# lingya/titan

Hardware: AMD Instinct MI355X
Metric: BFS GTEPS + PageRank s/iter, RMAT scale-24 (1 GPU) and scale-27 (1/2/4/8 GPU) (higher is better)
Workload: dtype int32 (BFS levels); f64 (PageRank)

## Files before the change

titan_amd/csrc/api_msbfs.cpp:

```cpp
#include <algorithm>
#include <cstdio>
#include <cstring>
#include "ctx.hpp"

using namespace tgo;

namespace tgo {

int ms_alloc(tgo_ctx* ctx) {
    Scratch& s = ctx->sc;
    if (s.ms_vis) return TGO_OK;
    const int64_t n = ctx->g.n;
    HIP_TRY(dev_alloc(ctx, s.ms_vis, n + 1));
    HIP_TRY(dev_alloc(ctx, s.ms_fr, n + 1));
    HIP_TRY(dev_alloc(ctx, s.ms_nx, n + 1));
    HIP_TRY(dev_alloc(ctx, s.ms_lvl, n * kLevelPlanes + 1));
    s.ms_clean = 0;
    if (n > ctx->g.n_active)
        for (int k = 0; k < kLevelPlanes; ++k)
            HIP_TRY(hipMemsetAsync(s.ms_lvl + static_cast<int64_t>(k) * n + ctx->g.n_active, 0,
                                   (n - ctx->g.n_active) * sizeof(uint64_t), ctx->stream));
    HIP_TRY(dev_alloc(ctx, s.ms_fbm, (n + 63) / 64 + 1));
    HIP_TRY(dev_alloc(ctx, s.ms_seeds, TGO_MAX_SOURCES));
    HIP_TRY(dev_alloc(ctx, s.ms_stat, 2 * TGO_MAX_SOURCES));
    HIP_TRY(dev_alloc(ctx, s.ms_srcent, TGO_MAX_SOURCES));
    ctx->st.device_bytes = ctx->dev_bytes;
    return TGO_OK;
}

double ms_split_of(const tgo_ctx* ctx) {
    static const double env = env_double("TGO_MS_SPLIT", 0.005);
    return tuned(ctx->tune.f64(TGO_TUNE_MS_SPLIT), env);
}
double ms_stay_of(const tgo_ctx* ctx) {
    static const double env = env_clamped("TGO_MS_STAY", kMsStayDefault, 0.0, HUGE_VAL);
    return tuned(ctx->tune.f64(TGO_TUNE_MS_STAY), env);
}
double ms_sparse_of(const tgo_ctx* ctx) {
    static const double env = env_clamped("TGO_MS_SPARSE", kMsSparseDefault, 0.0, HUGE_VAL);
    return tuned(ctx->tune.f64(TGO_TUNE_MS_SPARSE), env);
}
int64_t ms_head_of(const tgo_ctx* ctx) {
    static const int64_t env = static_cast<int64_t>(
        env_clamped("TGO_MS_HEAD", static_cast<double>(kMsHeadDefault), 0.0, static_cast<double>(kMsHeadMax)));
    return tuned(ctx->tune.i64(TGO_TUNE_MS_HEAD), env);
}

}

static int ms_cold_layout(tgo_ctx* ctx, int32_t scope, const View& pull, int64_t hot_req) {
    DevGraph& g = ctx->g;
    Scratch& s = ctx->sc;
    static const int64_t hot_env = static_cast<int64_t>(env_double("TGO_MS_COLD_HOT", 393216.0));
    static const int64_t seg_env = static_cast<int64_t>(env_double("TGO_MS_COLD_SEG", 393216.0));
    const int64_t hot = hot_req > 1 ? hot_req : hot_env, seg = hot_req > 1 ? hot_req : seg_env;
    if (g.msc_scope == scope && g.msc_req == hot) return TGO_OK;
// ... 10 lines not shown
    if (C == 0) return TGO_OK;
    adopt(ctx, g.msc_adj, cadj);
    adopt(ctx, g.msc_row, crow);
    if (!s.ms_cacc) {
        HIP_TRY(dev_alloc(ctx, s.ms_cacc, g.n + 1));
        HIP_TRY(dev_alloc(ctx, s.ms_need, g.n + 1));
        HIP_TRY(hipMemsetAsync(s.ms_need, 0, g.n + 1, ctx->stream));
    }
    g.msc_C = C;
    g.msc_hot = static_cast<int32_t>(hot);
    ctx->st.device_bytes = ctx->dev_bytes;
    return TGO_OK;
}

namespace tgo {

int run_ms_sweep(tgo_ctx* ctx, const int64_t* in, int32_t nseeds, int32_t max_depth, int32_t scope, int32_t flags) {
    int rc = TGO_OK;
    DevGraph& g = ctx->g;
    Scratch& s = ctx->sc;
    hipStream_t st = ctx->stream;
    const int64_t n = g.n;
    const View pull = pull_view(g, scope), push = push_view(g, scope);
    std::vector<int32_t> uniq;
    for (int r = 0; r < nseeds; ++r)
        if (std::find(uniq.begin(), uniq.end(), static_cast<int32_t>(in[r])) == uniq.end())
            uniq.push_back(static_cast<int32_t>(in[r]));
    s.ms_nsrc = nseeds;
    HIP_TRY(hipEventRecord(ctx->ev0, st));
    HIP_TRY(hipMemcpyAsync(s.ms_seeds, in, nseeds * sizeof(int64_t), hipMemcpyHostToDevice, st));
    HIP_TRY(hipMemcpyAsync(s.q[0], uniq.data(), uniq.size() * sizeof(int32_t), hipMemcpyHostToDevice, st));
    HIP_TRY(hipMemsetAsync(s.ms_vis, 0, n * 8, st));
    const bool masks_zero = s.ms_masks_zero;
    s.ms_masks_zero = false;
    if (!masks_zero) HIP_TRY(hipMemsetAsync(s.ms_fr, 0, n * 8, st));
    s.ms_nplanes = 0;
    HIP_TRY(k_ms_seed(s.ms_seeds, nseeds, s.ms_vis, s.ms_fr, INT64_MAX, st));
    HIP_TRY(k_degree_i64(push, s.q[0], static_cast<int64_t>(uniq.size()), s.qdeg, st));
    const uint64_t full = nseeds == 64 ? ~0ULL : ((1ULL << nseeds) - 1ULL);
    const int64_t total = pull.nlists > 1 ? g.out.nnz + g.in.nnz : (scope == TGO_SCOPE_IN_E ? g.out.nnz : g.in.nnz);
    static const double ms_alpha = env_double("TGO_MS_ALPHA", 12.0);
    static const bool trace = trace_on();
    static const int32_t filter_from = env_double("TGO_MS_FILTER", 0.0) != 0.0
        ? 0 : static_cast<int32_t>(env_double("TGO_MS_FILTER_FROM", -1.0));
    const bool filter = filter_from >= 0 && filter_from < n;
    const double split_frac = tgo::ms_split_of(ctx);
    const double stay_gamma = tgo::ms_stay_of(ctx), sparse_frac = tgo::ms_sparse_of(ctx);
    const int64_t head = tgo::ms_head_of(ctx);
    static const bool diag = env_double("TGO_MS_DIAG", 0.0) != 0.0;
    static const bool compact_on = env_i64("TGO_MS_COMPACT", 1) != 0 && !diag;
    static const int32_t compact_chunk = [] {
        const int64_t c = env_i64("TGO_MS_CHUNK", kMsChunkDefault);
        return static_cast<int32_t>(c == 512 || c == 1024 || c == 2048 ? c : kMsChunkDefault);
    }();
    int64_t qlen = static_cast<int64_t>(uniq.size());
    int64_t mf = 0;
    int64_t reached = qlen;
    bool srcent_ready = false;
    static const double push_light = env_double("TGO_MS_PUSH_LIGHT", 1.0 / 16.0);
    static const bool push_probe = env_double("TGO_MS_PUSH_PROBE", 1.0) != 0.0;
    static const int push_range_log2 = static_cast<int>(env_double("TGO_MS_PUSH_RANGE", 0.0));
    static const int64_t push_range_min = static_cast<int64_t>(env_double("TGO_MS_PUSH_RANGE_MIN", 1048576.0));
    const int depth = std::min(max_depth, 65534);
    uint64_t* fr = s.ms_fr;
    uint64_t* nx = s.ms_nx;
    int cur = 0, levels = 0;
    bool queued = true;
    bool pulled = false;
    bool cnt_zero = false;
    bool nx_clean = masks_zero;
    int64_t prev_mf = 0;
    int64_t mu = -1;
    bool level0_sparse = false, last_sparse = false;
    unsigned long long se_pub[TGO_MAX_SOURCES] = {};
    const volatile unsigned long long* hw = host_words(ctx);
    for (int L = 0; L < depth && qlen > 0; ++L) {
        const bool stay = pulled && mu >= 0 && stay_gamma > 0.0 &&
                          static_cast<double>(mu) <= stay_gamma * static_cast<double>(mf);
        const bool use_pull = stay || static_cast<double>(mf) * ms_alpha > static_cast<double>(total);
        DevSpan span(st, "msbfs.level", {"level", L}, {"pull", use_pull ? 1 : 0}, {"compact", 0});
        if ((rc = ms_planes_for(ctx, L + 1, true))) return rc;
        const uint32_t was_clean = s.ms_clean & ms_planes_written(L + 1);
        s.ms_clean &= ~was_clean;
        const bool queued_before = queued;
        if (!use_pull && !queued) {
            if (!cnt_zero) HIP_TRY(hipMemsetAsync(s.cnt, 0, sizeof(Counters), st));
            HIP_TRY(k_ms_queue(push, g.n_active, fr, s.q[cur], s.qdeg, s.cnt, st));
        }
        queued = !use_pull;
        const bool prev_pull = pulled;
        pulled = use_pull;
        bool sums = false;
        if (!use_pull && !queued_before) cnt_zero = false;
        bool sparse_level = false;
        bool count_open = false;
        if (use_pull) {
            if (!cnt_zero) HIP_TRY(hipMemsetAsync(s.cnt, 0, sizeof(Counters), st));
            cnt_zero = true;
            uint64_t sparse = 0;
            if (split_frac > 0.0 && !prev_pull) {
                static const bool srcent_check = env_double("TGO_MS_SRCENT_CHECK", 0.0) != 0.0;
                if (srcent_ready && srcent_check) {
                    HIP_TRY(k_ms_source_entries(push, fr, g.n_active, full, s.ms_stat, st));
                    unsigned long long x[TGO_MAX_SOURCES];
                    HIP_TRY(hipMemcpyAsync(x, s.ms_stat, sizeof(x), hipMemcpyDeviceToHost, st));
                    HIP_TRY(hipStreamSynchronize(st));
// ... 15 lines not shown
                std::sort(order, order + nseeds, [&](int a, int b) { return se[a] < se[b]; });
                const double budget = split_frac * static_cast<double>(total);
                double used = 0.0;
                for (int i = 0; i < nseeds; ++i) {
                    const int r = order[i];
                    if (used + static_cast<double>(se[r]) > budget) break;
                    used += static_cast<double>(se[r]);
                    sparse |= 1ULL << r;
                }
                if (sparse == full) sparse = 0;
                if (sparse) {
                    bool any = false;
                    for (int r = 0; r < nseeds; ++r) any |= ((sparse >> r) & 1ULL) && se[r] > 0;
                    if (!nx_clean) HIP_TRY(hipMemsetAsync(nx, 0, g.n_active * 8, st));
                    if (any) {
                        HIP_TRY(k_ms_queue(push, g.n_active, fr, s.q[cur ^ 1], s.qdeg, s.cnt, st, sparse));
                        if ((rc = turn(ctx))) return rc;
                        const int64_t sq = static_cast<int64_t>(s.hcnt->qlen);
                        if (sq > 0) {
                            if ((rc = scan_frontier(ctx, sq))) return rc;
                            HIP_TRY(k_ms_push(push, s.q[cur ^ 1], s.qpre, sq, fr, s.ms_vis, nx, st, PackTouch{}, sparse));
                        }
                    }
                    if (trace) std::fprintf(stderr, "[tgo] ms level %d split: %d sparse sources, %.0f push entries\n", L,
                                            __builtin_popcountll(sparse), used);
                }
            }
            if (filter) HIP_TRY(k_ms_fbitmap(fr, n, s.ms_fbm, st));
            MsColdSplit cs;
            static const bool cold_env = env_double("TGO_MS_COLD", 0.0) != 0.0;
            const int64_t cold = ctx->tune.i64(TGO_TUNE_MS_COLD);
            const bool cold_on = tuned_on(cold, cold_env);
            if (cold_on && !prev_pull && !filter) {
                if ((rc = ms_cold_layout(ctx, scope, pull, cold))) return rc;
                if (g.msc_C > 0) {
                    cs.hot_lim = g.msc_hot;
                    cs.acc = s.ms_cacc;
                    cs.need = s.ms_need;
                }
            }
            count_open = stay_gamma > 0.0 && !cs.acc && mf < prev_mf;
            const bool compact = compact_on && count_open && !sparse;
            if (compact) span.set_third(1);
            HIP_TRY(k_ms_pull(pull, push, g.n_active, full, fr, filter ? s.ms_fbm : nullptr, s.ms_vis, nx,
                              ms_planes(ctx), s.cnt, L + 1, st, filter ? filter_from : 0, full & ~sparse,
                              sparse ? nx : nullptr, cs, count_open, cs.acc ? 0 : head,
                              compact ? compact_chunk : 0));
            if (cs.acc) {
                HIP_TRY(k_ms_cold(g.msc_adj, g.msc_row, g.msc_C, fr, s.ms_need, s.ms_cacc, st));
                HIP_TRY(k_ms_finish(push, g.n_active, full, s.ms_vis, nx, sparse ? nx : nullptr, ms_planes(ctx), s.cnt,
                                    L + 1, s.ms_need, s.ms_cacc, st));
            }
        } else {
            HIP_TRY(k_level_prep(cnt_zero ? nullptr : s.cnt, nx, nx_clean ? 0 : g.n_active, s.qdeg + qlen, st));
            cnt_zero = true;
            const int64_t rng = static_cast<int64_t>(1) << std::min(40, std::max(0, push_range_log2));
            const int64_t nr = (g.n_active + rng - 1) / rng;
            const bool ranged = push_range_log2 > 0 && mf >= push_range_min && nr > 1 &&
                                (nr + 1) * qlen <= kMsRangePairs && nr * qlen + 1 <= n + 2;
            sparse_level = sparse_frac > 0.0 && !ranged &&
                           (L == 0 || static_cast<double>(mf) <= sparse_frac * static_cast<double>(g.n_active));
            sums = split_frac > 0.0 && (L == 0 || static_cast<double>(mf) * ms_alpha * 64.0 > static_cast<double>(total));
            if (ranged) {
                for (int b = 0; b < 2; ++b)
                    if (!s.ms_rp[b]) HIP_TRY(dev_alloc(ctx, s.ms_rp[b], kMsRangePairs));
                const bool light = static_cast<double>(reached) < push_light * static_cast<double>(n);
                HIP_TRY(k_ms_push_ranged(push, s.q[cur], qlen, g.n_active, rng, s.ms_rp[0], s.ms_rp[1], s.qdeg, s.qpre,
                                         s.cub_tmp, s.cub_bytes, fr, light ? nullptr : s.ms_vis, nx, st));
            } else {
            HIP_TRY(scan_exclusive_i64(s.cub_tmp, s.cub_bytes, s.qdeg, s.qpre, qlen + 1, st));
            if (sparse_level)
                HIP_TRY(k_ms_push_sparse(push, s.q[cur], s.qpre, qlen, fr, s.ms_vis, nx, s.q[cur ^ 1], s.cnt, st));
            else {
            const bool light = static_cast<double>(reached) < push_light * static_cast<double>(n);
            HIP_TRY(k_ms_push(push, s.q[cur], s.qpre, qlen, fr, light ? nullptr : s.ms_vis, nx, st, PackTouch{}, ~0ULL,
                              light ? push_probe : true));
            }
            }
            if (sums && !s.ms_srcent_zero) HIP_TRY(hipMemsetAsync(s.ms_srcent, 0, 64 * sizeof(unsigned long long), st));
            if (sums) s.ms_srcent_zero = false;
            const bool next_pull = static_cast<double>(mf) * ms_alpha * 8.0 > static_cast<double>(total);
            if (sparse_level) {
                HIP_TRY(k_ms_settle_sparse(push, s.q[cur ^ 1], s.qdeg, s.ms_vis, nx, ms_planes(ctx), s.cnt, L + 1, st,
                                           sums ? s.ms_srcent : nullptr, s.q[cur], qlen, fr));
            } else if (next_pull) {
                HIP_TRY(k_ms_settle_count(push, g.n_active, s.ms_vis, nx, ms_planes(ctx), s.cnt, L + 1, st,
                                          sums ? s.ms_srcent : nullptr));
                queued = false;
            } else {
                HIP_TRY(k_ms_settle(push, g.n_active, s.ms_vis, nx, ms_planes(ctx), s.q[cur ^ 1], s.qdeg, s.cnt, L + 1,
                                    st, sums ? s.ms_srcent : nullptr));
            }
        }
        srcent_ready = !use_pull && sums;
        {
            unsigned long long seq = 0;
            if ((rc = turn_begin(ctx, seq, sums ? s.ms_srcent : nullptr))) return rc;
            cnt_zero = true;
            if (sums) s.ms_srcent_zero = true;
            if (L + 1 < depth && (rc = ms_planes_for(ctx, L + 2, true))) return rc;
            if ((rc = wait_publish(ctx, seq))) return rc;
        }
        qlen = static_cast<int64_t>(s.hcnt->qlen);
        if (qlen == 0) s.ms_clean |= was_clean;
        prev_mf = mf;
        mf = static_cast<int64_t>(s.hcnt->mf);
        mu = count_open ? static_cast<int64_t>(s.hcnt->open) : -1;
        if (sums)
            for (int r = 0; r < TGO_MAX_SOURCES; ++r) se_pub[r] = hw[kPublishExtra + r];
        reached += qlen;
        nx_clean = sparse_level;
        last_sparse = sparse_level;
        if (L == 0) level0_sparse = sparse_level;
        if (trace) std::fprintf(stderr, "[tgo] ms level %d %s -> %lld vertices, %lld entries, %llu source-bits%s\n", L,
                                use_pull ? "pull" : "push", (long long)qlen, (long long)mf, s.hcnt->red[0],
                                use_pull ? (stay ? " (stayed in pull)" : "") : (sparse_level ? " (sparse)" : ""));
        if (trace && count_open) std::fprintf(stderr, "[tgo]   %lld list entries of still-open vertices\n", (long long)mu);
        if (trace && diag && use_pull) {
            unsigned long long d[kMsDiagWords] = {};
            HIP_TRY(k_ms_diag_take(d, st));
            std::fprintf(stderr, "[tgo]   pull: %llu entries examined, %llu hot / %llu cold mask gathers, %llu open vertices, "
                         "%llu stopped early; long lists: %llu, %llu entries examined (%llu hot / %llu cold gathers), "
                         "%llu stopped early\n", d[0], d[1], d[2], d[3], d[4], d[6], d[5], d[8], d[9], d[7]);
            std::fprintf(stderr, "[tgo]   long lists covered within 4 / 8 / 16 / 32 / 64 entries: %llu / %llu / %llu / %llu / %llu, "
                         "later %llu, never %llu (head %lld)\n", d[10], d[11], d[12], d[13], d[14], d[15], d[16],
                         static_cast<long long>(head));
        }
        std::swap(fr, nx);
        cur ^= 1;
        ++levels;
    }
    if (qlen > 0 && max_depth > depth)
        return fail(ctx, TGO_E_UNSUPPORTED, "multi-source BFS stores levels as uint16: depth > 65534");
    if (int rc = program_end(ctx, max_depth)) return rc;
    ctx->st.levels = levels;
    s.ms_masks_zero = level0_sparse && last_sparse && qlen == 0;
    if (flags & TGO_FLAG_STATS) {
        HIP_TRY(hipMemsetAsync(s.ms_stat, 0, 2 * TGO_MAX_SOURCES * sizeof(unsigned long long), st));
        HIP_TRY(k_ms_reach(pull, s.ms_vis, n, nseeds, s.ms_stat, s.ms_stat + TGO_MAX_SOURCES, st));
        HIP_TRY(hipStreamSynchronize(st));
    }
    return TGO_OK;
}

// ... 61 lines not shown
```

titan_amd/csrc/engine.hpp:

```cpp
#pragma once
#include <algorithm>
#include <cstdint>
#include <string>
#include <vector>
#include <hip/hip_runtime_api.h>
#include "../../include/titan_gpu_olap.h"
#include "env.hpp"

namespace tgo {

template <class T>
struct DevArray {
    T* p = nullptr;
    int64_t n = -1;
    DevArray() = default;
    DevArray(const DevArray&) = delete;
    DevArray& operator=(const DevArray&) = delete;
    DevArray(DevArray&& o) noexcept : p(o.p), n(o.n) { o.p = nullptr; o.n = -1; }
    DevArray& operator=(DevArray&& o) noexcept {
        if (this != &o) { reset(); p = o.p; n = o.n; o.p = nullptr; o.n = -1; }
        return *this;
    }
    ~DevArray() { reset(); }
    void reset() { if (p) (void)hipFree(p); p = nullptr; n = -1; }
// ... 621 lines not shown
                          const unsigned long long* offs, unsigned long long* cursor, int64_t* send, hipStream_t s);
hipError_t k_ds_mark_sizes(unsigned long long* counts, int nranks, int64_t qlen, unsigned long long* offs,
                           unsigned long long* cursor, const long long* track, int64_t* sizes, hipStream_t s);
hipError_t k_ds_apply(const View& push, const int64_t* recv, int64_t npairs, int64_t* dist, uint64_t* pend, int32_t* qn,
                      int64_t* qdeg_n, Counters* cnt, int64_t thr, const int64_t* ws_off, const int64_t* light,
                      long long* track, hipStream_t s);
hipError_t k_unpermute_i64(const int64_t* in, const int32_t* perm, int64_t* out, int64_t n, hipStream_t s);
hipError_t k_ms_seed(const int64_t* seeds, int nseeds, uint64_t* vis, uint64_t* fr, int64_t fr_rows, hipStream_t s);
constexpr int kMsDiagWords = 17;
hipError_t k_ms_diag_take(unsigned long long* out, hipStream_t s);
hipError_t k_ms_pull(const View& pull, const View& push, int64_t n_active, uint64_t full, const uint64_t* fr,
                     const uint64_t* fbm, uint64_t* vis, uint64_t* nx, LevelPlanes lvl, Counters* cnt,
                     int32_t next_level, hipStream_t s, int32_t filter_from, uint64_t dense = ~0ULL,
                     const uint64_t* cand = nullptr, MsColdSplit cs = MsColdSplit(), bool count_open = false,
                     int64_t head = 0, int32_t compact_chunk = 0);
hipError_t k_ms_cold(const int32_t* cadj, const int32_t* crow, int64_t C, const uint64_t* fr, const uint8_t* need,
                     uint64_t* acc, hipStream_t s);
hipError_t k_ms_finish(const View& push, int64_t n_active, uint64_t full, uint64_t* vis, uint64_t* nx,
                       const uint64_t* cand, LevelPlanes lvl, Counters* cnt, int32_t next_level, uint8_t* need,
                       const uint64_t* acc, hipStream_t s);
hipError_t k_cold_flags(const int32_t* adj, int64_t m, int32_t hot, uint32_t* flag, hipStream_t s);
hipError_t k_cold_emit(const int64_t* off, int64_t n, const int32_t* adj, int64_t m, const uint32_t* flag,
                       const uint64_t* pos, int64_t base, int32_t hot, int64_t seg, uint64_t* key, int32_t* val,
                       hipStream_t s);
hipError_t k_low_rows(const uint64_t* key, int64_t m, int32_t* row, hipStream_t s);
int build_ms_cold(const View& v, int64_t n, int32_t hot, int64_t seg, DevArray<int32_t>& cadj, DevArray<int32_t>& crow,
                  int64_t& C, hipStream_t s, std::string& err);
hipError_t k_ms_source_counts(const uint64_t* fr, int64_t n_active, unsigned long long* out64, hipStream_t s);
hipError_t k_ms_source_entries(const View& push, const uint64_t* fr, int64_t n_active, uint64_t cand,
                               unsigned long long* out64, hipStream_t s);
hipError_t k_ms_fbitmap(const uint64_t* fr, int64_t n, uint64_t* fbm, hipStream_t s);
hipError_t k_ms_queue(const View& push, int64_t n_active, const uint64_t* fr, int32_t* qn, int64_t* qdeg, Counters* cnt,
                      hipStream_t s, uint64_t mask = ~0ULL);
struct PackTouch { uint8_t* flag = nullptr; int64_t n_local = 1; int64_t cps = 1; };
hipError_t k_ms_push(const View& push, const int32_t* q, const int64_t* qpre, int64_t qlen, const uint64_t* fr,
                     const uint64_t* vis, uint64_t* nx, hipStream_t s, PackTouch touch = {}, uint64_t mask = ~0ULL,
                     bool probe = true, uint64_t* own_nx = nullptr, int64_t own_lo = 0);
constexpr double kMsStayDefault = 4.0;
constexpr double kMsSparseDefault = 1.0 / 16.0;
constexpr int64_t kMsHeadDefault = 4;
constexpr int64_t kMsHeadMax = 1 << 20;
constexpr int64_t kMsChunkDefault = 1024;
hipError_t k_ms_push_sparse(const View& push, const int32_t* q, const int64_t* qpre, int64_t qlen, const uint64_t* fr,
                            const uint64_t* vis, uint64_t* nx, int32_t* qn, Counters* cnt, hipStream_t s);
hipError_t k_ms_settle_sparse(const View& push, const int32_t* qn, int64_t* qdeg, uint64_t* vis, const uint64_t* nx,
                              LevelPlanes lvl, Counters* cnt, int32_t next_level, hipStream_t s,
                              unsigned long long* srcent, const int32_t* qp, int64_t qplen, uint64_t* fr);
constexpr int64_t kMsRangePairs = int64_t(1) << 22;
hipError_t k_ms_push_ranged(const View& push, const int32_t* q, int64_t qlen, int64_t n_active, int64_t S,
                            int64_t* P0, int64_t* P1, int64_t* cnt, int64_t* pre, void*& tmp, size_t& tmp_bytes,
                            const uint64_t* fr, const uint64_t* vis, uint64_t* nx, hipStream_t s, uint64_t mask = ~0ULL);
hipError_t k_ms_settle_count(const View& push, int64_t n_active, uint64_t* vis, uint64_t* nx, LevelPlanes lvl,
                            Counters* cnt, int32_t next_level, hipStream_t s, unsigned long long* srcent = nullptr);
hipError_t k_ms_settle(const View& push, int64_t n_active, uint64_t* vis, uint64_t* nx, LevelPlanes lvl, int32_t* qn,
                       int64_t* qdeg, Counters* cnt, int32_t next_level, hipStream_t s,
                       unsigned long long* srcent = nullptr);
hipError_t k_ms_reach(const View& v, const uint64_t* vis, int64_t n_active, int nsrc, unsigned long long* reached,
                      unsigned long long* entries, hipStream_t s);
hipError_t k_ms_extract(LevelPlanes lvl, int nplanes, const uint64_t* vis, const int32_t* perm, int r, int64_t* dist,
                        int64_t n, hipStream_t s);
hipError_t k_or_slices(const uint64_t* recv, int nslices, int64_t n_local, uint64_t* out, hipStream_t s);
constexpr int64_t kPackChunk = 2048;
hipError_t k_ms_pack(bool write, uint64_t* cand, int64_t n_local, int64_t cps, int64_t nchunks, int64_t* cnt,
                     const int64_t* offs, int64_t* send, hipStream_t s, uint8_t* touched = nullptr, int self = -1);
hipError_t k_ms_or_local(uint64_t* cand_own, int64_t n_local, int64_t cps, uint8_t* touched_own, uint64_t* nx,
                         hipStream_t s);
hipError_t k_slice_elems(const int64_t* off, int64_t cps, int nranks, int64_t* out, hipStream_t s);
hipError_t k_ms_or_pairs(const int64_t* pairs, int64_t npairs, uint64_t* nx, hipStream_t s);
hipError_t k_ms_pack_fixed(uint64_t* cand, int64_t n_local, int64_t cps, int64_t nchunks, const int64_t* offs,
                           int nranks, int64_t cap, int64_t* send, int* ovf, uint8_t* touched, hipStream_t s,
                           int self = -1);
hipError_t k_ms_or_fixed(const int64_t* recv, int nslices, int64_t cap, uint64_t* nx, hipStream_t s);
hipError_t k_part_td_mark(const View& push, const int32_t* q, const int64_t* qpre, int64_t qlen,
                          uint64_t* disc, const uint64_t* vb_local, int64_t lo, int64_t n_local, hipStream_t s);
hipError_t k_part_claim(const View& push, const uint64_t* recv, int nslices, int64_t words, int64_t n_local,
                        uint64_t* vb, uint64_t* nb, int32_t* level, int32_t* qn, int64_t* qdeg_n,
                        Counters* cnt, int32_t next_level, hipStream_t s, bool or_into_nb = false);
hipError_t k_part_td_claim(const View& push, const int32_t* q, const int64_t* qpre, int64_t qlen, uint64_t* disc,
                           uint64_t* vb, uint64_t* nb, int32_t* level, int32_t* qn, int64_t* qdeg_n, Counters* cnt,
                           int32_t next_level, int64_t lo, int64_t n_local, hipStream_t s);
int part_bfs_td_fused(tgo_ctx* ctx, int32_t level, uint64_t* disc, uint64_t* nb_local);
int part_bfs_claim_remote(tgo_ctx* ctx, int32_t level, const uint64_t* recv, int32_t nslices, uint64_t* nb_local);
int part_bfs_level_done(tgo_ctx* ctx);
hipError_t k_unpermute_i32(const int32_t* in, const int32_t* perm, int32_t* out, int64_t n, hipStream_t s);

hipError_t k_cc_init(int32_t* parent, int64_t n, hipStream_t s);
hipError_t k_cc_hook(const DevCsr& list, int64_t n, int64_t from, int64_t to, int32_t* parent, hipStream_t s);
hipError_t k_cc_jump(int32_t* parent, int64_t n, unsigned long long* changed, hipStream_t s);
hipError_t k_cc_scatter_ids(const int64_t* row_ids, const int32_t* perm, int64_t* tid, int64_t n, hipStream_t s);
hipError_t k_cc_min_id(const int32_t* parent, const int64_t* tid, int64_t n, int64_t* minid, hipStream_t s);
hipError_t k_cc_label(const int32_t* parent, const int64_t* minid, int64_t n, int64_t* label, unsigned long long* roots,
                      hipStream_t s);
hipError_t k_cc_pull_round(const View& pull, int64_t n, int64_t* label, unsigned long long* changed, hipStream_t s);
hipError_t k_cc_count_own(const int64_t* label, const int64_t* tid, int64_t n, unsigned long long* roots, hipStream_t s);

constexpr int64_t kTriLdsEntries = 16384;
hipError_t k_tri_fwd_count(const DevCsr& out, const DevCsr& in, int64_t n, int64_t* fcnt, int64_t* deg,
                           unsigned long long* max_fwd, hipStream_t s);
hipError_t k_tri_fwd_fill(const DevCsr& out, const DevCsr& in, int64_t n, const int64_t* foff, int32_t* fadj,
                          hipStream_t s);
hipError_t k_tri_count(const int64_t* foff, const int32_t* fadj, int64_t n, int64_t wave_row, int64_t block_row,
                       int64_t max_fwd, int64_t* tri, int32_t* blist, int32_t* wlist, unsigned long long* q,
                       hipStream_t s);
hipError_t k_tri_finish(const int64_t* tri, const int64_t* deg, int64_t n, double* lcc, unsigned long long* tot,
                        hipStream_t s);

// ... 177 lines not shown
```

titan_amd/csrc/msbfs.hip:

```cpp
#include <algorithm>
#include <cstdlib>
#include <hip/hip_runtime.h>
#include "frontier.hpp"

namespace tgo {
namespace {

constexpr int kMaxSources = 64;

__device__ __forceinline__ int32_t view_entry(const View& v, int64_t u, int64_t o) {
    const int64_t b0 = v.off0[u];
    const int64_t d0 = v.off0[u + 1] - b0;
    return o < d0 ? v.adj0[b0 + o] : v.adj1[v.off1[u] + (o - d0)];
}

__device__ __forceinline__ void record_level(int64_t v, uint64_t fresh, int32_t level, const LevelPlanes& pl) {
    for (int k = 0; k < kLevelPlanes && (level >> k); ++k)
        if ((level >> k) & 1) pl.p[k * pl.stride + v] |= fresh;
}

__device__ __forceinline__ void count_flush(Counters* cnt, unsigned long long nv, unsigned long long mf,
                                            unsigned long long bits, unsigned long long mu = 0) {
    __shared__ unsigned long long s_nv[kWavesPerBlock], s_mf[kWavesPerBlock], s_bits[kWavesPerBlock], s_mu[kWavesPerBlock];
    for (int off = 32; off > 0; off >>= 1) {
        nv += __shfl_xor(nv, off, 64);
        mf += __shfl_xor(mf, off, 64);
        bits += __shfl_xor(bits, off, 64);
        mu += __shfl_xor(mu, off, 64);
    }
    if (lane() == 0) {
        s_nv[threadIdx.x >> 6] = nv; s_mf[threadIdx.x >> 6] = mf; s_bits[threadIdx.x >> 6] = bits;
        s_mu[threadIdx.x >> 6] = mu;
    }
    __syncthreads();
    if (threadIdx.x == 0) {
        unsigned long long a = 0, m = 0, c = 0, u = 0;
        for (int w = 0; w < kWavesPerBlock; ++w) { a += s_nv[w]; m += s_mf[w]; c += s_bits[w]; u += s_mu[w]; }
        if (a) atomicAdd(&cnt->qlen, a);
        if (m) atomicAdd(&cnt->mf, m);
        if (c) atomicAdd(&cnt->red[0], c);
        if (u) atomicAdd(&cnt->open, u);
    }
}

__global__ void ms_seed(const int64_t* __restrict__ seeds, int nseeds, uint64_t* vis, uint64_t* fr, int64_t fr_rows) {
    const int r = static_cast<int>(threadIdx.x);
    if (blockIdx.x != 0 || r >= nseeds) return;
    const int64_t s = seeds[r];
    if (s < 0) return;
    atomicOr(reinterpret_cast<unsigned long long*>(&vis[s]), 1ULL << r);
    if (s < fr_rows) atomicOr(reinterpret_cast<unsigned long long*>(&fr[s]), 1ULL << r);
}

constexpr int64_t kCoop = 64;
__device__ __forceinline__ bool in_frontier(const uint64_t* __restrict__ fbm, int32_t u) {
    return !fbm || ((fbm[u >> 6] >> (u & 63)) & 1ULL);
// ... 705 lines not shown
                if (commit) {
                    nx[v] = fresh;
                    if (fresh) { vis[v] = seen | fresh; record_level(v, fresh, next_level, lvl); }
                }
            }
        }
        t[0] = {fresh != 0, static_cast<int32_t>(v), fresh ? push_degree(push, v) : 0};
        if (commit && srcent && __ballot(fresh != 0)) source_columns_add(fresh, static_cast<unsigned long long>(t[0].deg), ssum);
        return __ballot(c != 0) != 0;
    };
    chunk_extract<1>(words, probe, qn, qdeg, cnt);
    if (srcent) source_sums_flush(ssum, srcent);
}

__global__ void __launch_bounds__(kBlock) ms_settle_count(View push, int64_t n_active, uint64_t* __restrict__ vis,
        uint64_t* __restrict__ nx, LevelPlanes lvl, Counters* cnt, int32_t next_level,
        unsigned long long* __restrict__ srcent) {
    unsigned long long nv = 0, mf = 0, bits = 0, ssum = 0;
    const int64_t words = (n_active + 63) >> 6;
    const int64_t nw = (static_cast<int64_t>(gridDim.x) * blockDim.x) >> 6;
    for (int64_t w0 = (static_cast<int64_t>(blockIdx.x) * blockDim.x + threadIdx.x) >> 6; w0 < words; w0 += 4 * nw) {
        uint64_t c[4];
#pragma unroll
        for (int u = 0; u < 4; ++u) {
            const int64_t v = ((w0 + u * nw) << 6) + lane();
            c[u] = (w0 + u * nw < words && v < n_active) ? nx[v] : 0;
        }
#pragma unroll
        for (int u = 0; u < 4; ++u) {
            if (!__ballot(c[u] != 0)) continue;
            const int64_t v = ((w0 + u * nw) << 6) + lane();
            uint64_t fresh = 0;
            int64_t deg = 0;
            if (c[u]) {
                const uint64_t seen = vis[v];
                fresh = c[u] & ~seen;
                nx[v] = fresh;
                if (fresh) {
                    vis[v] = seen | fresh;
                    record_level(v, fresh, next_level, lvl);
                    deg = push_degree(push, v);
                    ++nv;
                    mf += static_cast<unsigned long long>(deg);
                    bits += static_cast<unsigned long long>(__popcll(fresh));
                }
            }
            if (srcent && __ballot(fresh != 0)) source_columns_add(fresh, static_cast<unsigned long long>(deg), ssum);
        }
    }
    count_flush(cnt, nv, mf, bits);
    if (srcent) source_sums_flush(ssum, srcent);
}

__global__ void __launch_bounds__(kBlock) ms_queue(View push, int64_t n_active, const uint64_t* __restrict__ fr,
        int32_t* __restrict__ qn, int64_t* __restrict__ qdeg, Counters* cnt, uint64_t mask) {
    const int64_t words = (n_active + 63) >> 6;
    auto probe = [&](int64_t wd, Take* t, bool) -> bool {
        const int64_t v = (wd << 6) + lane();
        const bool take = v < n_active && (fr[v] & mask) != 0;
        t[0] = {take, static_cast<int32_t>(v), take ? push_degree(push, v) : 0};
        return __ballot(take) != 0;
    };
    chunk_extract<1>(words, probe, qn, qdeg, cnt);
}

__global__ void or_slices(const uint64_t* __restrict__ recv, int nslices, int64_t n_local, uint64_t* __restrict__ out) {
    for (int64_t i = blockIdx.x * (int64_t)blockDim.x + threadIdx.x; i < n_local; i += (int64_t)gridDim.x * blockDim.x) {
        uint64_t m = 0;
        for (int s = 0; s < nslices; ++s) m |= recv[static_cast<int64_t>(s) * n_local + i];
        out[i] = m;
    }
}

template <bool kWrite>
__global__ void __launch_bounds__(kBlock) ms_pack(uint64_t* __restrict__ cand, int64_t n_local, int64_t cps,
        int64_t nchunks, int64_t* __restrict__ cnt, const int64_t* __restrict__ offs, int64_t* __restrict__ send,
        uint8_t* __restrict__ touched, int self) {
    const int64_t c = (blockIdx.x * (int64_t)blockDim.x + threadIdx.x) >> 6;
    if (c >= nchunks) return;
    const int64_t r = c / cps, j = c - r * cps;
    if ((touched && !touched[c]) || r == self) {
        if (!kWrite && lane() == 0) cnt[c] = 0;
        return;
    }
    const int64_t w0 = r * n_local + j * kPackChunk;
    const int64_t w1 = r * n_local + min(n_local, (j + 1) * kPackChunk);
    int64_t base = kWrite ? offs[c] : 0;
    for (int64_t g = w0; g < w1; g += 64) {
        const int64_t i = g + lane();
        const uint64_t m = cand[i];
        const uint64_t bal = __ballot(m != 0);
        if (kWrite && m) {
            const int64_t p = base + __popcll(bal & ((1ULL << lane()) - 1ULL));
            send[2 * p] = i - r * n_local;
            send[2 * p + 1] = static_cast<int64_t>(m);
            cand[i] = 0;
        }
        base += __popcll(bal);
    }
    if (!kWrite && lane() == 0) cnt[c] = base;
    if (kWrite && touched && lane() == 0) touched[c] = 0;
}
__global__ void slice_elems(const int64_t* __restrict__ off, int64_t cps, int nranks, int64_t* __restrict__ out) {
    const int r = threadIdx.x;
    if (blockIdx.x == 0 && r < nranks) out[r] = 2 * (off[(r + 1) * cps] - off[r * cps]);
}
// ... 198 lines not shown
    return hipGetLastError();
}
hipError_t k_ms_fbitmap(const uint64_t* fr, int64_t n, uint64_t* fbm, hipStream_t s) {
    const int64_t words = (n + 63) / 64;
    ms_fbitmap<<<grid_for(words * 64, 8192), kBlock, 0, s>>>(fr, n, fbm);
    return hipGetLastError();
}
hipError_t k_ms_queue(const View& push, int64_t n_active, const uint64_t* fr, int32_t* qn, int64_t* qdeg, Counters* cnt,
                      hipStream_t s, uint64_t mask) {
    ms_queue<<<extract_grid((n_active + 63) / 64), kBlock, 0, s>>>(push, n_active, fr, qn, qdeg, cnt, mask);
    return hipGetLastError();
}
hipError_t k_ms_push(const View& push, const int32_t* q, const int64_t* qpre, int64_t qlen, const uint64_t* fr,
                     const uint64_t* vis, uint64_t* nx, hipStream_t s, PackTouch touch, uint64_t mask, bool probe,
                     uint64_t* own_nx, int64_t own_lo) {
    static const bool e8 = env_i64("TGO_MS_PUSH_E", 0) == 8;
    if (e8) ms_push<8><<<256 * 8, kBlock, 0, s>>>(push, q, qpre, qlen, fr, vis, nx, touch, mask, probe, own_nx, own_lo,
                                                  nullptr, nullptr);
    else ms_push<><<<256 * 8, kBlock, 0, s>>>(push, q, qpre, qlen, fr, vis, nx, touch, mask, probe, own_nx, own_lo,
                                              nullptr, nullptr);
    return hipGetLastError();
}
hipError_t k_ms_push_sparse(const View& push, const int32_t* q, const int64_t* qpre, int64_t qlen, const uint64_t* fr,
                            const uint64_t* vis, uint64_t* nx, int32_t* qn, Counters* cnt, hipStream_t s) {
    if (!vis || !qn || !cnt) return hipErrorInvalidValue;
    ms_push<4, true><<<256 * 8, kBlock, 0, s>>>(push, q, qpre, qlen, fr, vis, nx, PackTouch{}, ~0ULL, true, nullptr, 0, qn,
                                               cnt);
    return hipGetLastError();
}
hipError_t k_ms_settle_sparse(const View& push, const int32_t* qn, int64_t* qdeg, uint64_t* vis, const uint64_t* nx,
                              LevelPlanes lvl, Counters* cnt, int32_t next_level, hipStream_t s,
                              unsigned long long* srcent, const int32_t* qp, int64_t qplen, uint64_t* fr) {
    ms_settle_sparse<<<512, kBlock, 0, s>>>(push, qn, qdeg, vis, nx, lvl, cnt, next_level, srcent, qp, qplen, fr);
    return hipGetLastError();
}
hipError_t k_ms_push_ranged(const View& push, const int32_t* q, int64_t qlen, int64_t n_active, int64_t S,
                            int64_t* P0, int64_t* P1, int64_t* cnt, int64_t* pre, void*& tmp, size_t& tmp_bytes,
                            const uint64_t* fr, const uint64_t* vis, uint64_t* nx, hipStream_t s, uint64_t mask) {
    if (S < 1 || qlen < 1) return hipErrorInvalidValue;
    const int64_t R = (n_active + S - 1) / S;
    if (R < 1) return hipErrorInvalidValue;
    ms_range_bounds<<<grid_for(qlen * (R + 1), 2048), kBlock, 0, s>>>(push, q, qlen, R, S, P0, P1);
    ms_range_counts<<<grid_for(R * qlen + 1, 2048), kBlock, 0, s>>>(push, qlen, R, P0, P1, cnt);
    hipError_t e = scan_exclusive_i64(tmp, tmp_bytes, cnt, pre, R * qlen + 1, s);
    if (e != hipSuccess) return e;
    ms_push_ranged<<<256 * 8, kBlock, 0, s>>>(push, q, qlen, R, P0, P1, pre, fr, vis, nx, mask);
    return hipGetLastError();
}
hipError_t k_ms_settle_count(const View& push, int64_t n_active, uint64_t* vis, uint64_t* nx, LevelPlanes lvl,
                            Counters* cnt, int32_t next_level, hipStream_t s, unsigned long long* srcent) {
    ms_settle_count<<<grid_for(n_active, 2048), kBlock, 0, s>>>(push, n_active, vis, nx, lvl, cnt, next_level, srcent);
    return hipGetLastError();
}
hipError_t k_ms_settle(const View& push, int64_t n_active, uint64_t* vis, uint64_t* nx, LevelPlanes lvl, int32_t* qn,
                       int64_t* qdeg, Counters* cnt, int32_t next_level, hipStream_t s, unsigned long long* srcent) {
    ms_settle<<<extract_grid((n_active + 63) / 64), kBlock, 0, s>>>(push, n_active, vis, nx, lvl, qn, qdeg, cnt,
                                                                    next_level, srcent);
    return hipGetLastError();
}
hipError_t k_ms_reach(const View& v, const uint64_t* vis, int64_t n_active, int nsrc, unsigned long long* reached,
                      unsigned long long* entries, hipStream_t s) {
    ms_reach<<<grid_for(n_active, 2048), kBlock, 0, s>>>(v, vis, n_active, nsrc, reached, entries);
    return hipGetLastError();
}
hipError_t k_ms_pack(bool write, uint64_t* cand, int64_t n_local, int64_t cps, int64_t nchunks, int64_t* cnt,
                     const int64_t* offs, int64_t* send, hipStream_t s, uint8_t* touched, int self) {
    const unsigned blocks = static_cast<unsigned>((nchunks * 64 + kBlock - 1) / kBlock);
    if (write) ms_pack<true><<<blocks, kBlock, 0, s>>>(cand, n_local, cps, nchunks, cnt, offs, send, touched, self);
    else ms_pack<false><<<blocks, kBlock, 0, s>>>(cand, n_local, cps, nchunks, cnt, offs, send, touched, self);
    return hipGetLastError();
}
hipError_t k_ms_or_local(uint64_t* cand_own, int64_t n_local, int64_t cps, uint8_t* touched_own, uint64_t* nx,
                         hipStream_t s) {
    ms_or_local<<<static_cast<unsigned>((cps * 64 + kBlock - 1) / kBlock), kBlock, 0, s>>>(cand_own, n_local, cps,
                                                                                           touched_own, nx);
    return hipGetLastError();
}
hipError_t k_slice_elems(const int64_t* off, int64_t cps, int nranks, int64_t* out, hipStream_t s) {
    slice_elems<<<1, kBlock, 0, s>>>(off, cps, nranks, out);
    return hipGetLastError();
}
hipError_t k_ms_pack_fixed(uint64_t* cand, int64_t n_local, int64_t cps, int64_t nchunks, const int64_t* offs,
                           int nranks, int64_t cap, int64_t* send, int* ovf, uint8_t* touched, hipStream_t s, int self) {
    const int64_t threads = nchunks * 64;
    ms_pack_fixed<<<static_cast<unsigned>((threads + kBlock - 1) / kBlock), kBlock, 0, s>>>(cand, n_local, cps, nchunks, offs,
                                                                                           cap, send, ovf, touched, self);
    fixed_headers<<<1, 64, 0, s>>>(offs, cps, nranks, cap, send);
    return hipGetLastError();
}
hipError_t k_ms_or_fixed(const int64_t* recv, int nslices, int64_t cap, uint64_t* nx, hipStream_t s) {
    const int64_t total = static_cast<int64_t>(nslices) * cap;
    int64_t g = (total + kBlock - 1) / kBlock;
    g = std::max<int64_t>(1, std::min<int64_t>(g, 65536));
    ms_or_fixed<<<static_cast<unsigned>(g), kBlock, 0, s>>>(recv, nslices, cap, nx);
    return hipGetLastError();
}
hipError_t k_ms_or_pairs(const int64_t* pairs, int64_t npairs, uint64_t* nx, hipStream_t s) {
    if (npairs > 0) ms_or_pairs<<<grid_for(npairs, 4096), kBlock, 0, s>>>(pairs, npairs, nx);
    return hipGetLastError();
}
hipError_t k_or_slices(const uint64_t* recv, int nslices, int64_t n_local, uint64_t* out, hipStream_t s) {
    or_slices<<<grid_for(n_local, 4096), kBlock, 0, s>>>(recv, nslices, n_local, out);
    return hipGetLastError();
}
hipError_t k_ms_extract(LevelPlanes lvl, int nplanes, const uint64_t* vis, const int32_t* perm, int r, int64_t* dist,
                        int64_t n, hipStream_t s) {
// ... 6 lines not shown
```

Before: 5826.

## Add merge-based tiled push kernel for multi-source BFS pre-pull levels

Adds a fused push-and-settle kernel for levels where the next step switches to pull. It merges the sorted adjacency lists of frontier vertices per row tile, ORs source masks into an LDS tile, then settles visited, level and next masks in the same pass. This avoids the separate level prep, global atomics into nx, and the separate settle-count sweep. In exchange it adds per-tile binary and galloping searches across up to 4096 lists with one large block per CU, which may underuse the GPU or lose on skewed degree distributions.

```diff
diff --git a/titan_amd/csrc/api_msbfs.cpp b/titan_amd/csrc/api_msbfs.cpp
--- a/titan_amd/csrc/api_msbfs.cpp
+++ b/titan_amd/csrc/api_msbfs.cpp
@@ -2,6 +2,7 @@
 #include <cstdio>
 #include <cstring>
 #include "ctx.hpp"
+#include "ms_merge.hpp"
 
 using namespace tgo;
 
@@ -118,6 +119,19 @@
     static const int32_t compact_chunk = [] {
         const int64_t c = env_i64("TGO_MS_CHUNK", kMsChunkDefault);
         return static_cast<int32_t>(c == 512 || c == 1024 || c == 2048 ? c : kMsChunkDefault);
+    }();
+    const bool merge_on = env_i64("TGO_MS_MERGE", 1) != 0;
+    const int64_t merge_tile = [] {
+        const int64_t t = env_i64("TGO_MS_MERGE_TILE", kMsMergeTileDefault);
+        return t >= 64 && t <= kMsMergeTileMax && t % 64 == 0 ? t : kMsMergeTileDefault;
+    }();
+    const int64_t merge_runs = [] {
+        const int64_t r = env_i64("TGO_MS_MERGE_RUNS", kMsMergeRunsDefault);
+        return r >= 1 && r <= kMsMergeRunsMax ? r : kMsMergeRunsDefault;
+    }();
+    const int64_t merge_cost = [] {
+        const int64_t c = env_i64("TGO_MS_MERGE_COST", kMsMergeRowCost);
+        return c >= 0 && c <= (1 << 20) ? c : kMsMergeRowCost;
     }();
     int64_t qlen = static_cast<int64_t>(uniq.size());
     int64_t mf = 0;
@@ -239,8 +253,6 @@
                                     L + 1, s.ms_need, s.ms_cacc, st));
             }
         } else {
-            HIP_TRY(k_level_prep(cnt_zero ? nullptr : s.cnt, nx, nx_clean ? 0 : g.n_active, s.qdeg + qlen, st));
-            cnt_zero = true;
             const int64_t rng = static_cast<int64_t>(1) << std::min(40, std::max(0, push_range_log2));
             const int64_t nr = (g.n_active + rng - 1) / rng;
             const bool ranged = push_range_log2 > 0 && mf >= push_range_min && nr > 1 &&
@@ -248,6 +260,21 @@
             sparse_level = sparse_frac > 0.0 && !ranged &&
                            (L == 0 || static_cast<double>(mf) <= sparse_frac * static_cast<double>(g.n_active));
             sums = split_frac > 0.0 && (L == 0 || static_cast<double>(mf) * ms_alpha * 64.0 > static_cast<double>(total));
+            const bool next_pull = static_cast<double>(mf) * ms_alpha * 8.0 > static_cast<double>(total);
+            const bool merge = merge_on && !ranged && !sparse_level && next_pull &&
+                               static_cast<int64_t>(push.nlists) * qlen <= kMsMergeLists && mf < INT32_MAX;
+            if (sums && !s.ms_srcent_zero) HIP_TRY(hipMemsetAsync(s.ms_srcent, 0, 64 * sizeof(unsigned long long), st));
+            if (sums) s.ms_srcent_zero = false;
+            if (merge) {
+                Span mspan("msbfs.merge_push", {"level", L}, {"lists", static_cast<int64_t>(push.nlists) * qlen});
+                if (!cnt_zero) HIP_TRY(hipMemsetAsync(s.cnt, 0, sizeof(Counters), st));
+                cnt_zero = true;
+                HIP_TRY(k_ms_push_merge(push, pull, s.q[cur], qlen, g.n_active, fr, s.ms_vis, nx, ms_planes(ctx), s.cnt,
+                                        L + 1, st, sums ? s.ms_srcent : nullptr, merge_tile, merge_runs, merge_cost));
+                queued = false;
+            } else {
+            HIP_TRY(k_level_prep(cnt_zero ? nullptr : s.cnt, nx, nx_clean ? 0 : g.n_active, s.qdeg + qlen, st));
+            cnt_zero = true;
             if (ranged) {
                 for (int b = 0; b < 2; ++b)
                     if (!s.ms_rp[b]) HIP_TRY(dev_alloc(ctx, s.ms_rp[b], kMsRangePairs));
@@ -264,9 +291,6 @@
                               light ? push_probe : true));
             }
             }
-            if (sums && !s.ms_srcent_zero) HIP_TRY(hipMemsetAsync(s.ms_srcent, 0, 64 * sizeof(unsigned long long), st));
-            if (sums) s.ms_srcent_zero = false;
-            const bool next_pull = static_cast<double>(mf) * ms_alpha * 8.0 > static_cast<double>(total);
             if (sparse_level) {
                 HIP_TRY(k_ms_settle_sparse(push, s.q[cur ^ 1], s.qdeg, s.ms_vis, nx, ms_planes(ctx), s.cnt, L + 1, st,
                                            sums ? s.ms_srcent : nullptr, s.q[cur], qlen, fr));
@@ -277,6 +301,7 @@
             } else {
                 HIP_TRY(k_ms_settle(push, g.n_active, s.ms_vis, nx, ms_planes(ctx), s.q[cur ^ 1], s.qdeg, s.cnt, L + 1,
                                     st, sums ? s.ms_srcent : nullptr));
+            }
             }
         }
         srcent_ready = !use_pull && sums;
diff --git a/titan_amd/csrc/engine.hpp b/titan_amd/csrc/engine.hpp
--- a/titan_amd/csrc/engine.hpp
+++ b/titan_amd/csrc/engine.hpp
@@ -697,6 +697,10 @@
                             const uint64_t* fr, const uint64_t* vis, uint64_t* nx, hipStream_t s, uint64_t mask = ~0ULL);
 hipError_t k_ms_settle_count(const View& push, int64_t n_active, uint64_t* vis, uint64_t* nx, LevelPlanes lvl,
                             Counters* cnt, int32_t next_level, hipStream_t s, unsigned long long* srcent = nullptr);
+hipError_t k_ms_push_merge(const View& push, const View& bal, const int32_t* q, int64_t qlen, int64_t n_active,
+                           const uint64_t* fr, uint64_t* vis, uint64_t* nx, LevelPlanes lvl, Counters* cnt,
+                           int32_t next_level, hipStream_t s, unsigned long long* srcent, int64_t tile, int64_t runs,
+                           int64_t row_cost);
 hipError_t k_ms_settle(const View& push, int64_t n_active, uint64_t* vis, uint64_t* nx, LevelPlanes lvl, int32_t* qn,
                        int64_t* qdeg, Counters* cnt, int32_t next_level, hipStream_t s,
                        unsigned long long* srcent = nullptr);
diff --git a/titan_amd/csrc/ms_merge.hpp b/titan_amd/csrc/ms_merge.hpp
--- /dev/null
+++ b/titan_amd/csrc/ms_merge.hpp
@@ -0,0 +1,83 @@
+#pragma once
+#include <cstdint>
+
+#if defined(__HIPCC__)
+#define TGO_MERGE_HD __host__ __device__ __forceinline__
+#else
+#define TGO_MERGE_HD inline
+#endif
+
+namespace tgo {
+
+constexpr int kMsMergeLists = 4096;
+constexpr int64_t kMsMergeTileDefault = 4096;
+constexpr int64_t kMsMergeTileMax = 4096;
+constexpr int64_t kMsMergeRunsDefault = 1024;
+constexpr int64_t kMsMergeRunsMax = 65536;
+constexpr int64_t kMsMergeRowCost = 64;
+
+TGO_MERGE_HD int64_t merge_cost(const int64_t* off0, const int64_t* off1, int nlists, int64_t row, int64_t c) {
+    int64_t x = off0[row] - off0[0] + c * row;
+    if (nlists > 1) x += off1[row] - off1[0];
+    return x;
+}
+
+TGO_MERGE_HD int64_t merge_run_boundary(const int64_t* off0, const int64_t* off1, int nlists, int64_t n_active,
+                                        int64_t R, int64_t c, int64_t b) {
+    const int64_t words = (n_active + 63) >> 6;
+    if (b <= 0) return 0;
+    if (b >= R) return words;
+    const int64_t total = merge_cost(off0, off1, nlists, n_active, c);
+    const int64_t target = total / R * b + total % R * b / R;
+    int64_t lo = 0, hi = words;
+    while (lo < hi) {
+        const int64_t w = (lo + hi) >> 1;
+        const int64_t row = (w << 6) < n_active ? (w << 6) : n_active;
+        if (merge_cost(off0, off1, nlists, row, c) >= target) hi = w; else lo = w + 1;
+    }
+    return lo;
+}
+
+TGO_MERGE_HD void merge_run_bounds(const int64_t* off0, const int64_t* off1, int nlists, int64_t n_active, int64_t R,
+                                   int64_t c, int64_t b, int64_t& lo, int64_t& hi) {
+    lo = merge_run_boundary(off0, off1, nlists, n_active, R, c, b) << 6;
+    hi = merge_run_boundary(off0, off1, nlists, n_active, R, c, b + 1) << 6;
+    if (hi > n_active) hi = n_active;
+    if (lo > hi) lo = hi;
+}
+
+struct MergeSeek {
+    int32_t lo, hi, step;
+    int32_t at;
+    TGO_MERGE_HD void start(int32_t span, bool gallop) {
+        lo = 0; hi = span; step = gallop ? 1 : 0; at = INT32_MAX;
+    }
+    TGO_MERGE_HD int32_t probe() {
+        if (hi - lo <= 1) return -1;
+        if (step > 0) {
+            if (step < hi - lo) return lo + step;
+            step = 0;
+        }
+        return lo + ((hi - lo) >> 1);
+    }
+    TGO_MERGE_HD void take(int32_t p, int32_t x, int32_t key) {
+        if (x < key) {
+            lo = p;
+            if (step > 0) step <<= 1;
+        } else {
+            hi = p;
+            at = x;
+            step = 0;
+        }
+    }
+};
+
+TGO_MERGE_HD int64_t merge_seek(const int32_t* adj, int64_t lo, int64_t hi, int32_t key, bool gallop, int32_t& at) {
+    MergeSeek s;
+    s.start(static_cast<int32_t>(hi - lo), gallop);
+    for (int32_t p; (p = s.probe()) >= 0;) s.take(p, adj[lo + p], key);
+    at = s.at;
+    return lo + s.hi;
+}
+
+}
diff --git a/titan_amd/csrc/msbfs.hip b/titan_amd/csrc/msbfs.hip
--- a/titan_amd/csrc/msbfs.hip
+++ b/titan_amd/csrc/msbfs.hip
@@ -2,6 +2,7 @@
 #include <cstdlib>
 #include <hip/hip_runtime.h>
 #include "frontier.hpp"
+#include "ms_merge.hpp"
 
 namespace tgo {
 namespace {
@@ -813,6 +814,239 @@
     if (srcent) source_sums_flush(ssum, srcent);
 }
 
+constexpr int kMergeThreads = 1024;
+constexpr int kMergeWaves = kMergeThreads / 64;
+constexpr int kMergeLists = kMsMergeLists / kMergeThreads;
+constexpr int kMergeE = 4;
+constexpr int kMergeSettle = 4;
+__global__ void __launch_bounds__(kMergeThreads) ms_push_merge(View push, const int64_t* __restrict__ bal0, const int64_t* __restrict__ bal1,
+        int bal_lists, const int32_t* __restrict__ q,
+        int32_t qlen, int64_t n_active, const uint64_t* __restrict__ fr, uint64_t* __restrict__ vis,
+        uint64_t* __restrict__ nx, LevelPlanes lvl, Counters* cnt, int32_t next_level,
+        unsigned long long* __restrict__ srcent, int32_t T, int64_t R, int64_t row_cost) {
+    __shared__ uint64_t s_tile[kMsMergeTileMax];
+    __shared__ uint64_t s_mask[kMsMergeLists];
+    __shared__ int64_t s_pos[kMsMergeLists];
+    __shared__ int32_t s_rem[kMsMergeLists];
+    __shared__ int32_t s_next[kMsMergeLists];
+    __shared__ int32_t s_pre[kMsMergeLists + 1];
+    __shared__ int32_t s_wave[kMergeWaves];
+    const int tid = static_cast<int>(threadIdx.x);
+    const int wave = tid >> 6;
+    const int nl = push.nlists > 1 ? 2 * qlen : qlen;
+    unsigned long long nv = 0, mf = 0, bits = 0, ssum = 0;
+    for (int i = tid; i < kMsMergeTileMax; i += kMergeThreads) s_tile[i] = 0;
+    for (int64_t run = blockIdx.x; run < R; run += gridDim.x) {
+        int64_t row_lo, row_hi;
+        merge_run_bounds(bal0, bal1, bal_lists, n_active, R, row_cost, run, row_lo, row_hi);
+        if (row_lo >= row_hi) continue;
+        __syncthreads();
+        {
+            MergeSeek sk[kMergeLists];
+            const int32_t* ap[kMergeLists];
+            int64_t beg[kMergeLists];
+            int32_t span[kMergeLists];
+            uint64_t msk[kMergeLists];
+#pragma unroll
+            for (int k = 0; k < kMergeLists; ++k) {
+                const int j = tid * kMergeLists + k;
+                const bool live = j < nl;
+                const bool l1 = live && j >= qlen;
+                const int32_t u = q[live ? (l1 ? j - qlen : j) : 0];
+                const int64_t* off = l1 ? push.off1 : push.off0;
+                const int64_t b = off[u], e = off[u + 1];
+                beg[k] = b - 1;
+                ap[k] = (l1 ? push.adj1 : push.adj0) + beg[k];
+                span[k] = live ? static_cast<int32_t>(e - b) + 1 : 1;
+                msk[k] = live ? fr[u] : 0;
+                sk[k].start(span[k], false);
+            }
+            const int32_t key = static_cast<int32_t>(row_lo);
+            for (;;) {
+                int32_t p[kMergeLists];
+                bool any = false;
+#pragma unroll
+                for (int k = 0; k < kMergeLists; ++k) { p[k] = sk[k].probe(); any |= p[k] >= 0; }
+                if (!any) break;
+                int32_t x[kMergeLists];
+#pragma unroll
+                for (int k = 0; k < kMergeLists; ++k) x[k] = *(p[k] >= 0 ? ap[k] + p[k] : q);
+#pragma unroll
+                for (int k = 0; k < kMergeLists; ++k)
+                    if (p[k] >= 0) sk[k].take(p[k], x[k], key);
+            }
+#pragma unroll
+            for (int k = 0; k < kMergeLists; ++k) {
+                const int j = tid * kMergeLists + k;
+                s_pos[j] = beg[k] + sk[k].hi;
+                s_rem[j] = span[k] - sk[k].hi;
+                s_next[j] = sk[k].at;
+                s_mask[j] = msk[k];
+            }
+        }
+        __syncthreads();
+        for (int64_t tile_lo = row_lo; tile_lo < row_hi; tile_lo += T) {
+            const int64_t tile_hi = min(tile_lo + T, row_hi);
+            const int32_t rows = static_cast<int32_t>(tile_hi - tile_lo);
+            int32_t len[kMergeLists];
+            {
+                MergeSeek sk[kMergeLists];
+                const int32_t* ap[kMergeLists];
+                bool act[kMergeLists];
+                int64_t pos[kMergeLists];
+                int32_t rem[kMergeLists];
+#pragma unroll
+                for (int k = 0; k < kMergeLists; ++k) {
+                    const int j = tid * kMergeLists + k;
+                    act[k] = static_cast<int64_t>(s_next[j]) < tile_hi;
+                    pos[k] = s_pos[j];
+                    rem[k] = s_rem[j];
+                    ap[k] = ((push.nlists > 1 && j >= qlen) ? push.adj1 : push.adj0) + pos[k];
+                    sk[k].start(act[k] ? rem[k] : 0, true);
+                }
+                const int32_t key = static_cast<int32_t>(min(tile_hi, static_cast<int64_t>(INT32_MAX)));
+                for (;;) {
+                    int32_t p[kMergeLists];
+                    bool any = false;
+#pragma unroll
+                    for (int k = 0; k < kMergeLists; ++k) { p[k] = sk[k].probe(); any |= p[k] >= 0; }
+                    if (!any) break;
+                    int32_t x[kMergeLists];
+#pragma unroll
+                    for (int k = 0; k < kMergeLists; ++k) x[k] = *(p[k] >= 0 ? ap[k] + p[k] : q);
+#pragma unroll
+                    for (int k = 0; k < kMergeLists; ++k)
+                        if (p[k] >= 0) sk[k].take(p[k], x[k], key);
+                }
+#pragma unroll
+                for (int k = 0; k < kMergeLists; ++k) {
+                    const int j = tid * kMergeLists + k;
+                    len[k] = 0;
+                    if (act[k]) {
+                        len[k] = sk[k].hi;
+                        s_pos[j] = pos[k] + sk[k].hi;
+                        s_rem[j] = rem[k] - len[k];
+                        s_next[j] = sk[k].at;
+                    }
+                }
+            }
+            int32_t mine = 0;
+#pragma unroll
+            for (int k = 0; k < kMergeLists; ++k) mine += len[k];
+            int32_t incl = mine;
+            for (int o = 1; o < 64; o <<= 1) {
+                const int32_t y = __shfl_up(incl, o, 64);
+                if (lane() >= o) incl += y;
+            }
+            if (lane() == 63) s_wave[wave] = incl;
+            __syncthreads();
+            int32_t before = 0, total = 0;
+#pragma unroll
+            for (int w = 0; w < kMergeWaves; ++w) {
+                const int32_t x = s_wave[w];
+                if (w < wave) before += x;
+                total += x;
+            }
+            int32_t run_pre = before + incl - mine;
+#pragma unroll
+            for (int k = 0; k < kMergeLists; ++k) {
+                s_pre[tid * kMergeLists + k] = run_pre;
+                run_pre += len[k];
+            }
+            if (tid == kMergeThreads - 1) s_pre[kMsMergeLists] = total;
+            __syncthreads();
+            for (int64_t base = 0; base < total; base += kMergeThreads * kMergeE) {
+                int32_t v[kMergeE];
+                int own[kMergeE];
+                const int32_t* src[kMergeE];
+#pragma unroll
+                for (int k = 0; k < kMergeE; ++k) {
+                    const int32_t g = static_cast<int32_t>(base) + k * kMergeThreads + tid;
+                    src[k] = q;
+                    own[k] = -1;
+                    if (g >= total) continue;
+                    int a = 0, b = kMsMergeLists;
+                    while (b - a > 1) { const int c = (a + b) >> 1; if (s_pre[c] <= g) a = c; else b = c; }
+                    const int32_t* adj = (push.nlists > 1 && a >= qlen) ? push.adj1 : push.adj0;
+                    src[k] = adj + (s_pos[a] - (s_pre[a + 1] - g));
+                    own[k] = a;
+                }
+#pragma unroll
+                for (int k = 0; k < kMergeE; ++k) v[k] = *src[k];
+#pragma unroll
+                for (int k = 0; k < kMergeE; ++k) {
+                    if (own[k] < 0) continue;
+                    const int64_t r = static_cast<int64_t>(v[k]) - tile_lo;
+                    const uint64_t m = s_mask[own[k]];
+                    if (m && r >= 0 && r < rows) atomicOr(reinterpret_cast<unsigned long long*>(&s_tile[r]), m);
+                }
+            }
+            __syncthreads();
+            if (total == 0) {
+                for (int32_t i = tid; i < rows; i += kMergeThreads) nx[tile_lo + i] = 0;
+            } else {
+                const int32_t tw = (rows + 63) >> 6;
+                for (int32_t wb = 0; wb < tw; wb += kMergeWaves * kMergeSettle) {
+                    uint64_t seen[kMergeSettle];
+#pragma unroll
+                    for (int u = 0; u < kMergeSettle; ++u) {
+                        const int32_t i = ((wb + u * kMergeWaves + wave) << 6) + lane();
+                        seen[u] = vis[tile_lo + (i < rows ? i : 0)];
+                    }
+                    static_assert(kMergeSettle == 4, "the select below");
+#pragma unroll 1
+                    for (int u = 0; u < kMergeSettle; ++u) {
+                        const int32_t w = wb + u * kMergeWaves + wave;
+                        if (w >= tw) break;
+                        const int32_t i = (w << 6) + lane();
+                        const int64_t vtx = tile_lo + i;
+                        const uint64_t sn = u == 0 ? seen[0] : u == 1 ? seen[1] : u == 2 ? seen[2] : seen[3];
+                        uint64_t fresh = 0;
+                        if (i < rows) {
+                            fresh = s_tile[i] & ~sn;
+                            s_tile[i] = 0;
+                            nx[vtx] = fresh;
+                        }
+                        int64_t deg = 0;
+                        if (fresh) {
+                            vis[vtx] = sn | fresh;
+                            record_level(vtx, fresh, next_level, lvl);
+                            deg = push_degree(push, vtx);
+                            ++nv;
+                            mf += static_cast<unsigned long long>(deg);
+                            bits += static_cast<unsigned long long>(__popcll(fresh));
+                        }
+                        if (srcent && __ballot(fresh != 0)) source_columns_add(fresh, static_cast<unsigned long long>(deg), ssum);
+                    }
+                }
+            }
+            __syncthreads();
+        }
+    }
+    __syncthreads();
+    unsigned long long* s_sum = reinterpret_cast<unsigned long long*>(s_pos);
+    for (int off = 32; off > 0; off >>= 1) {
+        nv += __shfl_xor(nv, off, 64);
+        mf += __shfl_xor(mf, off, 64);
+        bits += __shfl_xor(bits, off, 64);
+    }
+    if (lane() == 0) { s_sum[wave] = nv; s_sum[kMergeWaves + wave] = mf; s_sum[2 * kMergeWaves + wave] = bits; }
+    s_sum[(3 + wave) * 64 + lane()] = ssum;
+    __syncthreads();
+    if (tid == 0) {
+        unsigned long long a = 0, m = 0, c = 0;
+        for (int w = 0; w < kMergeWaves; ++w) { a += s_sum[w]; m += s_sum[kMergeWaves + w]; c += s_sum[2 * kMergeWaves + w]; }
+        if (a) atomicAdd(&cnt->qlen, a);
+        if (m) atomicAdd(&cnt->mf, m);
+        if (c) atomicAdd(&cnt->red[0], c);
+    }
+    if (srcent && tid < 64) {
+        unsigned long long t = 0;
+        for (int w = 0; w < kMergeWaves; ++w) t += s_sum[(3 + w) * 64 + tid];
+        if (t) atomicAdd(&srcent[tid], t);
+    }
+}
+
 __global__ void __launch_bounds__(kBlock) ms_queue(View push, int64_t n_active, const uint64_t* __restrict__ fr,
         int32_t* __restrict__ qn, int64_t* __restrict__ qdeg, Counters* cnt, uint64_t mask) {
     const int64_t words = (n_active + 63) >> 6;
@@ -1117,6 +1351,24 @@
     ms_settle_count<<<grid_for(n_active, 2048), kBlock, 0, s>>>(push, n_active, vis, nx, lvl, cnt, next_level, srcent);
     return hipGetLastError();
 }
+hipError_t k_ms_push_merge(const View& push, const View& bal, const int32_t* q, int64_t qlen, int64_t n_active,
+                           const uint64_t* fr, uint64_t* vis, uint64_t* nx, LevelPlanes lvl, Counters* cnt,
+                           int32_t next_level, hipStream_t s, unsigned long long* srcent, int64_t tile, int64_t runs,
+                           int64_t row_cost) {
+    if (qlen < 1 || push.nlists * qlen > kMsMergeLists || bal.nlists < 1 || tile < 64 || tile > kMsMergeTileMax ||
+        tile % 64 != 0 || runs < 1 || runs > kMsMergeRunsMax || row_cost < 0 || row_cost > (1 << 20) || n_active < 1)
+        return hipErrorInvalidValue;
+    static const int cus = [] {
+        int dev = 0, n = 0;
+        if (hipGetDevice(&dev) != hipSuccess || hipDeviceGetAttribute(&n, hipDeviceAttributeMultiprocessorCount, dev) != hipSuccess)
+            n = 0;
+        return n > 0 ? n : 256;
+    }();
+    const int grid = static_cast<int>(std::min<int64_t>(runs, cus));
+    ms_push_merge<<<grid, kMergeThreads, 0, s>>>(push, bal.off0, bal.off1, bal.nlists, q, static_cast<int32_t>(qlen), n_active, fr, vis, nx, lvl, cnt,
+                                                 next_level, srcent, static_cast<int32_t>(tile), runs, row_cost);
+    return hipGetLastError();
+}
 hipError_t k_ms_settle(const View& push, int64_t n_active, uint64_t* vis, uint64_t* nx, LevelPlanes lvl, int32_t* qn,
                        int64_t* qdeg, Counters* cnt, int32_t next_level, hipStream_t s, unsigned long long* srcent) {
     ms_settle<<<extract_grid((n_active + 63) / 64), kBlock, 0, s>>>(push, n_active, vis, nx, lvl, qn, qdeg, cnt,
```

New measurement: 5374. -7.8%, worse.
